# CGuerreroCordova/HydroDEM

Measured on AMD Instinct MI355X. Metric: Mcells/s sink-fill+D8 on 16384^2 float32 DEM, higher is better.
Workload: dtype f32; 1 GPU; 16384x16384 float32 synthetic DEM (SURVEY 8d 'rough': plane + 4 sinusoids + 0.5 m noise + 0.1% pits), SinkFill eps=0 to exact convergence + D8; 16384 rows per GPU, row-block partition; rows_per_gpu=16384, cols=16384, tiles=70225, visits_unchanged=25721, visits_flat=3352, certifying_rounds=0, halo_exchanges=0

## Files before the change

### hydrodem_amd/csrc/hdem_sinkfill.hip

```cpp
#include "hdem_internal.h"

#include <algorithm>
#include <cmath>
#include <cstdlib>

namespace {

constexpr int FT = 62;
constexpr int WN = 64;
constexpr int TS = WN + 1;
constexpr int NT = 64;
constexpr int ITER_MAX = 8;
constexpr int INIT_NT = 256;
constexpr int INIT_ROWS = 4;
constexpr int KEY_NONE = 0x7fffffff;
constexpr int SEED_KEYS = 1 << 20;
constexpr int AUX_SC1 = 16;
constexpr int COARSE_SHIFT = 4;
constexpr int HUB_EDGE = 4 * WN;
constexpr float HUB_BIG = 3.0e38f;
constexpr int HUB_MIN_TILES = 64;
constexpr int HUB_MIN_TILES_NESTED = 36;
constexpr int COARSE_MIN_CELLS = 6000 * 6000;
constexpr int PEND_SHARDS = 64;
// ... 131 lines not shown
        h_cur = h_next;
    }
}

__device__ __forceinline__ void transpose(float (&v)[WN], float *T, int lane)
{
#pragma unroll
    for (int i = 0; i < WN; ++i) T[i * TS + lane] = v[i];
    __syncthreads();
#pragma unroll
    for (int i = 0; i < WN; ++i) v[i] = T[lane * TS + i];
    __syncthreads();
}

__device__ __forceinline__ float wave_min(float v)
{
#pragma unroll
    for (int o = 32; o >= 1; o >>= 1) v = fminf(v, __shfl_xor(v, o));
    return v;
}

__device__ __forceinline__ int float_key(float f)
{
    int i = __builtin_bit_cast(int, f);
    return i ^ ((i >> 31) & 0x7fffffff);
}

#ifdef HDEM_VISIT_PROF
#define PROF_MARK(k) do { long long now_ = wall_clock64(); out.ticks[k] += now_ - tprof_; tprof_ = now_; } while (0)
#else
#define PROF_MARK(k) do { } while (0)
#endif

struct hub_bounds {
    float lv[9];
    bool mine;
};

struct visit_result {
#ifdef HDEM_VISIT_PROF
    long long ticks[6];
#endif
    bool changed;
    bool more;
    unsigned dirs;
    int iters;
    int flat_bits;
    int zmax_bits;
};

template <bool HAS_EPS, bool COHERENT>
__device__ __forceinline__ visit_result tile_visit(const float *__restrict__ zg, float *wg,
                                                   int H, int W, float eps, int ty, int tx,
                                                   float *T, uint8_t *d8 = nullptr,
                                                   float flat_level = HDEM_INF,
                                                   const hub_bounds *hb = nullptr)
{
    const int lane = threadIdx.x;
    const int y0 = ty * FT, x0 = tx * FT;
    const int x = x0 + lane;
#ifdef HDEM_VISIT_PROF
    const long long tprof_entry_ = wall_clock64();
#endif

    float z[WN], w[WN];
    const int xc = min(x, W - 1);
    float *wbase = wg + (size_t)y0 * W;
    const size_t wbytes = (size_t)(H - y0) * W * sizeof(float);
    const __amdgpu_buffer_rsrc_t wrsrc = __builtin_amdgcn_make_buffer_rsrc(
        wbase, 0, COHERENT ? (int)(unsigned)(wbytes < 0xffffffffull ? wbytes : 0xffffffffull) : 0,
        0x00020000);
    const int hbrow = H - 1 - y0;
    if (COHERENT) {
        const __amdgpu_buffer_rsrc_t zrsrc = __builtin_amdgcn_make_buffer_rsrc(
            const_cast<float *>(zg) + (size_t)y0 * W, 0,
            (int)(unsigned)(wbytes < 0xffffffffull ? wbytes : 0xffffffffull), 0x00020000);
        const unsigned col = (unsigned)xc * (unsigned)sizeof(float);
        const unsigned pitch = (unsigned)W * (unsigned)sizeof(float);
#pragma unroll
        for (int r = 0; r < WN; ++r) {
            const unsigned row = (unsigned)min(r, hbrow) * pitch;
            z[r] = __builtin_bit_cast(float, __builtin_amdgcn_raw_buffer_load_b32(zrsrc, col, row, 0));
            w[r] = __builtin_bit_cast(float, __builtin_amdgcn_raw_buffer_load_b32(wrsrc, col, row, AUX_SC1));
        }
    } else {
#pragma unroll
        for (int r = 0; r < WN; ++r) {
            const size_t o = (size_t)min(y0 + r, H - 1) * W + xc;
            z[r] = zg[o];
            w[r] = wg[o];
        }
    }
    const bool lane_pin = lane == 0 || lane == WN - 1 || x == 0 || x >= W - 1;
    const bool lane_out = x >= W;
    const bool partial = x0 + WN > W || y0 + WN > H;
    unsigned long long free_n = ~0ull, free_s = ~0ull;
    unsigned free_lo = 0, free_hi = 0;
    float hub_t = -HDEM_INF, hub_m = -HDEM_INF, hub_b = -HDEM_INF;
    if (COHERENT && hb) {
        const int k = lane == 0 ? 0 : (lane == WN - 1 ? 2 : 1);
        hub_t = k == 0 ? hb->lv[0] : (k == 1 ? hb->lv[1] : hb->lv[2]);
        hub_m = k == 0 ? hb->lv[3] : (k == 1 ? hb->lv[4] : hb->lv[5]);
        hub_b = k == 0 ? hb->lv[6] : (k == 1 ? hb->lv[7] : hb->lv[8]);
    }
    const int pin_from = lane_pin ? 0 : min(hbrow, WN - 1);
    const int raise_to = x >= W - 1 ? 0 : min(hbrow, WN);
#pragma unroll
    for (int r = 0; r < WN; ++r) {
        float wc = fminf(w[r], HDEM_INF), zc = fminf(z[r], HDEM_INF);
        if (COHERENT) {
            const float bound = r == 0 ? hub_t : (r == WN - 1 ? hub_b : hub_m);
            wc = fmaxf(wc, r < raise_to ? bound : -HDEM_INF);
        }
        if (!COHERENT && partial && (lane_out || y0 + r >= H)) { wc = HDEM_INF; zc = HDEM_INF; }
        if (COHERENT) {
            if (r == 0) free_n = __ballot(zc < wc);
            if (r == WN - 1) free_s = __ballot(zc < wc);
            if (r < 32) shift_in_less(free_lo, zc, wc);
            else shift_in_less(free_hi, zc, wc);
        }
        z[r] = (r == 0 || r == WN - 1 || r >= pin_from) ? wc : zc;
        w[r] = wc;
    }
    if (COHERENT && partial) {
        const unsigned long long in_lanes = __ballot(!lane_out);
        free_n &= in_lanes;
        free_s = hbrow >= WN - 1 ? (free_s & in_lanes) : 0ull;
    }

    if (COHERENT && flat_level < HDEM_INF) {
        const bool inner_lane = lane >= 2 && lane <= FT - 1;
#pragma unroll
        for (int r = 2; r <= FT - 1; ++r) w[r] = inner_lane ? flat_level : w[r];
    }

    unsigned long long free_w = 0, free_e = 0;
    if (COHERENT) {
        const unsigned wl = __builtin_amdgcn_readlane(free_lo, 0), wh = __builtin_amdgcn_readlane(free_hi, 0);
        const unsigned el = __builtin_amdgcn_readlane(free_lo, WN - 1), eh = __builtin_amdgcn_readlane(free_hi, WN - 1);
        free_w = ((unsigned long long)__builtin_bitreverse32(wh) << 32) | __builtin_bitreverse32(wl);
        free_e = ((unsigned long long)__builtin_bitreverse32(eh) << 32) | __builtin_bitreverse32(el);
        if (partial && hbrow < WN - 1) {
            const unsigned long long in_rows = (2ull << hbrow) - 1;
            free_w &= in_rows;
            free_e &= in_rows;
        }
    }
    visit_result out;
    out.flat_bits = out.zmax_bits = FLAT_NONE;
#ifdef HDEM_VISIT_PROF
    for (int k = 0; k < 6; ++k) out.ticks[k] = 0;
    long long tprof_ = tprof_entry_;
    asm volatile("s_waitcnt vmcnt(0)" ::: "memory");
    PROF_MARK(0);
#endif
    out.dirs = 0;
    out.iters = 0;
    scan_masks V = {0, 0, 0};
    check_rows<HAS_EPS>(z, w, eps, V);
    V.all |= V.first | V.last;
    bool more = V.all != 0;
    out.changed = more;
    const bool force_store = COHERENT && hb && hb->mine;
    const unsigned long long b1 = 1ull << 1, bl = 1ull << FT;
    unsigned long long mv_r1 = V.first, mv_r62 = V.last, mv_c1 = V.all & b1, mv_c62 = V.all & bl;
    PROF_MARK(1);
    if (more || force_store) {
        float zt[WN];
#pragma unroll
        for (int r = 0; r < WN; ++r) zt[r] = z[r];
        transpose(zt, T, lane);
        float r1_prev = w[1], r62_prev = w[FT];
        if (lane == 1 || lane == FT) {
            float *dst = T + (lane == 1 ? 0 : WN);
#pragma unroll
            for (int r = 0; r < WN; ++r) dst[r] = w[r];
        }
        __syncthreads();
        float c1_prev = T[lane], c62_prev = T[WN + lane];
        __syncthreads();
        float hl = HDEM_INF, hr = HDEM_INF;
        PROF_MARK(2);
        for (; out.iters < ITER_MAX && more; ++out.iters) {
            scan_lines<HAS_EPS>(z, w, eps);
            transpose(w, T, lane);
            hl = w[0];
            hr = w[WN - 1];
            or_changed(mv_c1, w[1], c1_prev);
            or_changed(mv_c62, w[FT], c62_prev);
            c1_prev = w[1];
            c62_prev = w[FT];
            scan_lines<HAS_EPS>(zt, w, eps);
            or_changed(mv_c1, w[1], c1_prev);
            or_changed(mv_c62, w[FT], c62_prev);
            c1_prev = w[1];
            c62_prev = w[FT];
// ... 299 lines not shown
                                                       bool changed, bool more, unsigned dirs,
                                                       int iters)
{
    const int lane = threadIdx.x;
    const int ty = t / tiles_x, tx = t - ty * tiles_x, slot = t / G, owner = t % G;
    int *my_state = state + (size_t)owner * S, *my_prio = prio + (size_t)owner * S;
    const int now_key = SEED_KEYS + (int)(wall_clock64() & 0x3fffffff);
    if (changed && dirs) {
        asm volatile("s_waitcnt vmcnt(0)" ::: "memory");
        if (lane < 8 && ((dirs >> lane) & 1u)) {
            const int t2 = neighbour_tile(lane, ty, tx, tiles_x, tiles_y);
            if (t2 >= 0) wake_async(t2, now_key, G, S, state, prio, pend);
        }
    }
    if (lane == 8) {
        if (more) atomicMin(&my_prio[slot], now_key);
        const int target = more ? ST_QUEUED : ST_IDLE;
        const int old = atomicCAS(&my_state[slot], ST_RUNNING, target);
        if (old == ST_DIRTY) atomicExch(&my_state[slot], ST_QUEUED);
        else if (target == ST_IDLE) atomicAdd(pend + (owner % PEND_SHARDS) * PEND_STRIDE, -1);
        add_stats(stats, b, changed, more, iters);
    }
}

struct flat_result {
    int handled;
    bool changed;
    unsigned dirs;
    float level;
};

__device__ __attribute__((noinline)) flat_result flat_visit(float *wg, int H, int W, int ty, int tx,
                                                            float L, float zmax,
                                                            const hub_bounds *hb)
{
    const int lane = threadIdx.x;
    const int y0 = ty * FT, x0 = tx * FT;
    float *wbase = wg + (size_t)y0 * W;
    const size_t wbytes = (size_t)(H - y0) * W * sizeof(float);
    const __amdgpu_buffer_rsrc_t wrsrc = __builtin_amdgcn_make_buffer_rsrc(
        wbase, 0, (int)(unsigned)(wbytes < 0xffffffffull ? wbytes : 0xffffffffull), 0x00020000);
    auto at = [&](int r, int c) { return (unsigned)(((size_t)r * W + x0 + c) * sizeof(float)); };
    auto ld = [&](unsigned off) {
        return fminf(__builtin_bit_cast(float, __builtin_amdgcn_raw_buffer_load_b32(
                         wrsrc, off, 0, AUX_SC1)), HDEM_INF);
    };
    float top = ld(at(0, lane)), bottom = ld(at(WN - 1, lane));
    float left = ld(at(lane, 0)), right = ld(at(lane, WN - 1));
    if (hb) {
        const int k = lane == 0 ? 0 : (lane == WN - 1 ? 2 : 1);
        top = fmaxf(top, k == 0 ? hb->lv[0] : (k == 1 ? hb->lv[1] : hb->lv[2]));
        bottom = fmaxf(bottom, k == 0 ? hb->lv[6] : (k == 1 ? hb->lv[7] : hb->lv[8]));
        left = fmaxf(left, k == 0 ? hb->lv[0] : (k == 1 ? hb->lv[3] : hb->lv[6]));
        right = fmaxf(right, k == 0 ? hb->lv[2] : (k == 1 ? hb->lv[5] : hb->lv[8]));
    }
    const float low = wave_min(fminf(fminf(top, bottom), fminf(left, right)));
    flat_result out = {1, false, 0u, L};
    if (low >= L) return out;
    if (low < zmax) { out.handled = 0; return out; }
    out.changed = true;
    out.level = low;
    const unsigned bits = __builtin_bit_cast(unsigned, low);
    if (lane >= 1 && lane <= FT) {
        __builtin_amdgcn_raw_buffer_store_b32(bits, wrsrc, at(1, lane), 0, AUX_SC1);
        __builtin_amdgcn_raw_buffer_store_b32(bits, wrsrc, at(FT, lane), 0, AUX_SC1);
        if (lane >= 2 && lane <= FT - 1) {
            __builtin_amdgcn_raw_buffer_store_b32(bits, wrsrc, at(lane, 1), 0, AUX_SC1);
            __builtin_amdgcn_raw_buffer_store_b32(bits, wrsrc, at(lane, FT), 0, AUX_SC1);
        }
    }
    const unsigned long long mid = ((1ull << FT) - 1) << 1, hi = 1ull << (WN - 1);
    const unsigned long long n = __ballot(top > low), s_ = __ballot(bottom > low);
    const unsigned long long w_ = __ballot(left > low), e = __ballot(right > low);
    if (n & 1ull) out.dirs |= 1u << 0;
    if (n & mid) out.dirs |= 1u << 1;
    if (n & hi) out.dirs |= 1u << 2;
    if (w_ & mid) out.dirs |= 1u << 3;
    if (e & mid) out.dirs |= 1u << 4;
    if (s_ & 1ull) out.dirs |= 1u << 5;
    if (s_ & mid) out.dirs |= 1u << 6;
    if (s_ & hi) out.dirs |= 1u << 7;
    return out;
}

__global__ __launch_bounds__(NT) void flat_store_kernel(float *wg, int H, int W, int tiles_x,
                                                        int ntiles, const int *__restrict__ flat,
                                                        const float *__restrict__ hub_lev,
                                                        const int *__restrict__ applied,
// ... 211 lines not shown
                                                          int *pend, int *error,
                                                          unsigned long long *stats,
                                                          long long budget_ticks, int soft,
                                                          int *flat, int *zmax,
                                                          const float *__restrict__ hub_lev,
                                                          int *applied,
                                                          const int *__restrict__ seam_words)
{
    __shared__ float T[WN * TS];
    if (seam_words && (seam_words[0] | seam_words[1] | seam_words[2]) == 0) return;
    const int G = gridDim.x, b = blockIdx.x;
    const long long t_begin = wall_clock64();
    if (threadIdx.x == 0) atomicAdd(error + 1, 1);
    while (ld_relaxed(error + 1) < G && ld_relaxed(error) == 0) {
        if (wall_clock64() - t_begin > 20000) {
            if (threadIdx.x == 0) atomicExch(error + 3, 1);
            break;
        }
        __builtin_amdgcn_s_sleep(8);
    }
    if (ld_relaxed(error) != 0) return;
    long long t_mark = t_begin, busy = 0, idle = 0;
    for (;;) {
        if (soft && wall_clock64() - t_begin > budget_ticks) break;
        const int t = __builtin_amdgcn_readfirstlane(
            async_pick(b, G, S, ntiles, state, prio, pend, soft ? error + 2 : error, t_begin,
                       budget_ticks));
        long long now = wall_clock64();
        idle += now - t_mark;
        t_mark = now;
        if (t < 0) break;
        const int ty = t / tiles_x, tx = t - ty * tiles_x;
        float flat_level = HDEM_INF;
        hub_bounds hb;
        bool use_hb = false, first_visit = false;
        const int fb_raw = HAS_EPS ? FLAT_NONE : ld_relaxed(flat + t);
        if (!HAS_EPS && hub_lev) {
            const int k9 = threadIdx.x < 9 ? (int)threadIdx.x : 4;
            const int ny = ty + k9 / 3 - 1, nx = tx + k9 % 3 - 1;
            const bool there = threadIdx.x < 9 && ny >= 0 && ny < tiles_y && nx >= 0 && nx < tiles_x;
            float l = -HDEM_INF;
            int seen = 1;
            if (there) {
                seen = ld_relaxed(applied + ny * tiles_x + nx);
                l = hub_lev[(size_t)(2 * ny + 1) * (2 * tiles_x + 1) + 2 * nx + 1];
            }
            l = (seen || l != l) ? -HDEM_INF : (l >= HUB_BIG ? HDEM_INF : l);
            first_visit = __builtin_amdgcn_readlane(seen, 4) == 0;
            use_hb = first_visit || __ballot(l > -HDEM_INF) != 0;
            if (use_hb) {
#pragma unroll
                for (int k = 0; k < 9; ++k)
                    hb.lv[k] = __builtin_bit_cast(
                        float, __builtin_amdgcn_readlane(__builtin_bit_cast(int, l), k));
                hb.mine = first_visit;
            }
            asm volatile("" ::: "memory");
        }
        if (!HAS_EPS) {
            const int fb = __builtin_amdgcn_readfirstlane(fb_raw);
            if (fb != FLAT_NONE) {
                flat_level = __builtin_bit_cast(float, fb);
                const float zm = __builtin_bit_cast(
                    float, __builtin_amdgcn_readfirstlane(ld_relaxed(zmax + t)));
                const flat_result f = flat_visit(wg, H, W, ty, tx, flat_level, zm,
                                                 use_hb ? &hb : nullptr);
                if (f.handled) {
                    if (f.changed) {
                        if (threadIdx.x == 0)
                            __hip_atomic_store(flat + t, __builtin_bit_cast(int, f.level),
                                               __ATOMIC_RELAXED, __HIP_MEMORY_SCOPE_AGENT);
                        asm volatile("s_waitcnt vmcnt(0)" ::: "memory");
                    }
                    async_finish(t, b, G, S, tiles_x, tiles_y, state, prio, pend, stats, f.changed,
                                 false, f.dirs, 0);
                    now = wall_clock64();
                    if (threadIdx.x == 8) {
                        stats[(size_t)b * STAT_WORDS + STAT_FLAT] += 1;
                        stats[(size_t)b * STAT_WORDS + STAT_FLAT_SAME] += f.changed ? 0 : 1;
                    }
                    busy += now - t_mark;
                    t_mark = now;
                    continue;
                }
            }
        }
        const visit_result v = tile_visit<HAS_EPS, true>(zg, wg, H, W, eps, ty, tx, T, nullptr,
                                                         flat_level, use_hb ? &hb : nullptr);
        if (first_visit) {
            asm volatile("s_waitcnt vmcnt(0)" ::: "memory");
            if (threadIdx.x == 0)
                __hip_atomic_store(applied + t, 1, __ATOMIC_RELAXED, __HIP_MEMORY_SCOPE_AGENT);
            asm volatile("s_waitcnt vmcnt(0)" ::: "memory");
        }
        if (!HAS_EPS && (v.flat_bits != FLAT_NONE || flat_level < HDEM_INF)) {
            if (threadIdx.x == 0) {
                __hip_atomic_store(flat + t, v.flat_bits, __ATOMIC_RELAXED, __HIP_MEMORY_SCOPE_AGENT);
                if (v.flat_bits != FLAT_NONE)
                    __hip_atomic_store(zmax + t, v.zmax_bits, __ATOMIC_RELAXED,
                                       __HIP_MEMORY_SCOPE_AGENT);
            }
            asm volatile("s_waitcnt vmcnt(0)" ::: "memory");
        }
#ifdef HDEM_VISIT_PROF
        const long long t_v = wall_clock64();
#endif
        async_finish(t, b, G, S, tiles_x, tiles_y, state, prio, pend, stats, v.changed, v.more,
                     v.dirs, v.iters);
        now = wall_clock64();
#ifdef HDEM_VISIT_PROF
        if (threadIdx.x == 8) {
            for (int k = 0; k < 6; ++k) stats[(size_t)b * STAT_WORDS + STAT_PROF + k] += v.ticks[k];
            stats[(size_t)b * STAT_WORDS + STAT_PROF + 6] += (unsigned long long)(now - t_v);
        }
#endif
        busy += now - t_mark;
        t_mark = now;
    }
    if (threadIdx.x == 0) {
        stats[(size_t)b * STAT_WORDS + 4] += (unsigned long long)busy;
        stats[(size_t)b * STAT_WORDS + 5] += (unsigned long long)idle;
// ... 824 lines not shown
```

### hydrodem_amd/csrc/hdem_stencil.hip

```cpp
#include "hdem_internal.h"

namespace {

constexpr int TW = 256;
constexpr int TH = 32;
template <typename T> struct tile_rows { static constexpr int value = sizeof(T) == 8 ? TH / 2 : TH; };
constexpr int LS = TW + 8;
constexpr int NT = 256;

__device__ __forceinline__ int reflect(int i, int n)
{
    while (i < 0 || i >= n) {
        if (i < 0) i = -i - 1;
        if (i >= n) i = 2 * n - 1 - i;
    }
    return i;
}

template <typename T, bool REFLECT>
__device__ __forceinline__ void stage_tile(const T *__restrict__ src, int H, int W,
                                           int y0, int x0, T *t)
{
    constexpr int THT = tile_rows<T>::value;
    constexpr int V = 16 / sizeof(T);
// ... 20 lines not shown
                int xx = gx + k;
                T e = T(0);
                if (REFLECT) e = src[(size_t)gy * W + reflect(xx, W)];
                else if (row_ok && xx < W) e = src[(size_t)gy * W + xx];
                v[j][k] = e;
            }
        }
    }
#pragma unroll
    for (int j = 0; j < CHUNKS; ++j) {
        const int i = tid + j * NT;
        if (i < (THT + 2) * CPR)
            *reinterpret_cast<vec_t *>(t + (i / CPR) * LS + 4 + (i % CPR) * V) = v[j];
    }
    for (int i = tid; i < (THT + 2) * 2; i += NT) {
        int r = i >> 1, side = i & 1;
        int gy = y0 - 1 + r, gx = side ? x0 + TW : x0 - 1;
        T e = T(0);
        if (REFLECT) e = src[(size_t)reflect(gy, H) * W + reflect(gx, W)];
        else if (gy >= 0 && gy < H && gx >= 0 && gx < W) e = src[(size_t)gy * W + gx];
        t[r * LS + (side ? 4 + TW : 3)] = e;
    }
}

template <typename T>
__device__ __forceinline__ void read_row6(const T *t, int r, int cg, T (&o)[6])
{
    const T *p = t + r * LS + 4 + 4 * cg;
    o[0] = p[-1];
    o[1] = p[0]; o[2] = p[1]; o[3] = p[2]; o[4] = p[3];
    o[5] = p[4];
}

__device__ __forceinline__ unsigned d8_code(float nw, float n, float ne, float w,
                                            float c, float e, float sw, float s,
                                            float se)
{
    const float dg = 0.70710678f;
    float best = 0.0f;
    unsigned code = 0;
    float d;
    d = (c - nw) * dg; if (d > best) { best = d; code = 32; }
    d = (c - n);       if (d > best) { best = d; code = 64; }
    d = (c - ne) * dg; if (d > best) { best = d; code = 128; }
    d = (c - w);       if (d > best) { best = d; code = 16; }
    d = (c - e);       if (d > best) { best = d; code = 1; }
    d = (c - sw) * dg; if (d > best) { best = d; code = 8; }
    d = (c - s);       if (d > best) { best = d; code = 4; }
    d = (c - se) * dg; if (d > best) { best = d; code = 2; }
    return code;
}

__global__ __launch_bounds__(NT) void d8_kernel(const float *__restrict__ z, int H,
                                               int W, uint8_t *__restrict__ out,
                                               int tiles_x, int vec_store)
{
    __shared__ __attribute__((aligned(16))) float t[(TH + 2) * LS];
    const int bx = blockIdx.x % tiles_x, by = blockIdx.x / tiles_x;
    const int x0 = bx * TW, y0 = by * TH;
    stage_tile<float, false>(z, H, W, y0, x0, t);
    __syncthreads();

    const int cg = threadIdx.x & 63, rg = threadIdx.x >> 6;
    const int x = x0 + 4 * cg;
    if (x >= W) return;
    float a[6], b[6], c[6];
    read_row6(t, rg * 8 + 0, cg, a);
    read_row6(t, rg * 8 + 1, cg, b);
#pragma unroll
    for (int rr = 0; rr < 8; ++rr) {
        const int y = y0 + rg * 8 + rr;
        read_row6(t, rg * 8 + rr + 2, cg, c);
        if (y < H) {
            unsigned code[4];
#pragma unroll
            for (int k = 0; k < 4; ++k) {
                unsigned cd = d8_code(a[k], a[k + 1], a[k + 2], b[k], b[k + 1],
                                      b[k + 2], c[k], c[k + 1], c[k + 2]);
                int xx = x + k;
                bool interior = y > 0 && y < H - 1 && xx > 0 && xx < W - 1;
                code[k] = interior ? cd : 0u;
            }
            uint8_t *o = out + (size_t)y * W + x;
            if (vec_store && x + 4 <= W) {
                *reinterpret_cast<uint32_t *>(o) =
                    code[0] | (code[1] << 8) | (code[2] << 16) | (code[3] << 24);
            } else {
#pragma unroll
                for (int k = 0; k < 4; ++k)
                    if (x + k < W) o[k] = (uint8_t)code[k];
            }
        }
#pragma unroll
        for (int k = 0; k < 6; ++k) { a[k] = b[k]; b[k] = c[k]; }
    }
}

template <bool HAS_EPS>
__global__ __launch_bounds__(NT) void certify_d8_kernel(const float *__restrict__ z,
                                                       const float *__restrict__ w, int H, int W,
                                                       float eps, uint8_t *__restrict__ out,
                                                       int tiles_x, int vec_store, int *flag)
{
    __shared__ __attribute__((aligned(16))) float t[(TH + 2) * LS];
    const int bx = blockIdx.x % tiles_x, by = blockIdx.x / tiles_x;
    const int x0 = bx * TW, y0 = by * TH;
    stage_tile<float, false>(w, H, W, y0, x0, t);
    __syncthreads();

    const int cg = threadIdx.x & 63, rg = threadIdx.x >> 6;
    const int x = x0 + 4 * cg;
    if (x >= W) return;
    float zc[8][4];
#pragma unroll
    for (int rr = 0; rr < 8; ++rr) {
        const int y = min(y0 + rg * 8 + rr, H - 1);
        if (x + 4 <= W) {
            const hdem_f4 m = hdem_ld4u(z + (size_t)y * W + x);
            zc[rr][0] = m[0]; zc[rr][1] = m[1]; zc[rr][2] = m[2]; zc[rr][3] = m[3];
        } else {
#pragma unroll
            for (int k = 0; k < 4; ++k) zc[rr][k] = z[(size_t)y * W + min(x + k, W - 1)];
        }
    }
    bool lower = false;
    float a[6], b[6], c[6];
    read_row6(t, rg * 8 + 0, cg, a);
    read_row6(t, rg * 8 + 1, cg, b);
#pragma unroll
    for (int rr = 0; rr < 8; ++rr) {
        const int y = y0 + rg * 8 + rr;
        read_row6(t, rg * 8 + rr + 2, cg, c);
        if (y < H) {
            unsigned code[4];
#pragma unroll
            for (int k = 0; k < 4; ++k) {
                const int xx = x + k;
                const bool interior = y > 0 && y < H - 1 && xx > 0 && xx < W - 1;
                float m = fminf(fminf(fminf(a[k], a[k + 1]), fminf(a[k + 2], b[k])),
                                fminf(fminf(b[k + 1], b[k + 2]), fminf(c[k], fminf(c[k + 1], c[k + 2]))));
                m = fminf(m, HDEM_INF);
                if (HAS_EPS) m += eps;
                const float wc = fminf(b[k + 1], HDEM_INF), zz = fminf(zc[rr][k], HDEM_INF);
                lower |= interior && __builtin_amdgcn_fmed3f(zz, wc, m) != wc;
                const unsigned cd = d8_code(a[k], a[k + 1], a[k + 2], b[k], b[k + 1], b[k + 2], c[k],
                                            c[k + 1], c[k + 2]);
                code[k] = interior ? cd : 0u;
            }
            if (out) {
                uint8_t *o = out + (size_t)y * W + x;
                if (vec_store && x + 4 <= W) {
                    *reinterpret_cast<uint32_t *>(o) =
                        code[0] | (code[1] << 8) | (code[2] << 16) | (code[3] << 24);
                } else {
#pragma unroll
                    for (int k = 0; k < 4; ++k)
                        if (x + k < W) o[k] = (uint8_t)code[k];
                }
            }
        }
#pragma unroll
        for (int k = 0; k < 6; ++k) { a[k] = b[k]; b[k] = c[k]; }
    }
    if (lower) *flag = 1;
}

template <typename T>
__device__ __forceinline__ T mean9(const T (&a)[6], const T (&b)[6], const T (&c)[6],
                                   int k, int do_round)
{
    double acc = 0.0;
    acc += (double)a[k]; acc += (double)a[k + 1]; acc += (double)a[k + 2];
    acc += (double)b[k]; acc += (double)b[k + 1]; acc += (double)b[k + 2];
    acc += (double)c[k]; acc += (double)c[k + 1]; acc += (double)c[k + 2];
    T s = (T)acc;
    T m = s / T(9);
    if (do_round) m = sizeof(T) == 4 ? (T)rintf((float)m) : (T)rint((double)m);
    return m;
}

template <typename T>
__global__ __launch_bounds__(NT) void boxmean3_kernel(const T *__restrict__ x, int H,
                                                     int W, T *__restrict__ out,
                                                     int tiles_x, int do_round)
{
    constexpr int THT = tile_rows<T>::value;
    constexpr int RPW = THT / 4;
    __shared__ __attribute__((aligned(16))) T t[(THT + 2) * LS];
    const int bx = blockIdx.x % tiles_x, by = blockIdx.x / tiles_x;
    const int x0 = bx * TW, y0 = by * THT;
    stage_tile<T, true>(x, H, W, y0, x0, t);
    __syncthreads();

    const int cg = threadIdx.x & 63, rg = threadIdx.x >> 6;
    const int xc = x0 + 4 * cg;
    if (xc >= W) return;
    T a[6], b[6], c[6];
// ... 38 lines not shown
    double acc = 0.0;
    for (int j = 0; j < kh; ++j) {
        int gy = reflect(y + j - py, H);
        for (int k = 0; k < kw; ++k) {
            double w = wt[(kh - 1 - j) * kw + (kw - 1 - k)];
            if (w != 0.0)
                acc += (double)x[(size_t)gy * W + reflect(xx + k - px, W)] * w;
        }
    }
    const T s = (T)acc;
    out[i] = s / (T)(kh * kw);
}

template <typename T>
__global__ __launch_bounds__(NT) void around_kernel(const T *x, int64_t n, T *out)
{
    int64_t i = (int64_t)blockIdx.x * NT + threadIdx.x;
    if (i < n) out[i] = sizeof(T) == 4 ? (T)rintf((float)x[i]) : (T)rint((double)x[i]);
}

inline int tiles_of(int H, int W, int th, int *tx)
{
    *tx = (W + TW - 1) / TW;
    return *tx * ((H + th - 1) / th);
}

}

int hdem_certify_d8_launch(hdem_ctx *ctx, const float *z, const float *w, int H, int W, float eps,
                           uint8_t *d8, int *flag)
{
    int tx, nt = tiles_of(H, W, TH, &tx);
    const int vec = d8 && (W % 4 == 0) && ((uintptr_t)d8 % 4 == 0);
    if (eps != 0.0f)
        hipLaunchKernelGGL(certify_d8_kernel<true>, dim3(nt), dim3(NT), 0, ctx->stream, z, w, H, W,
                           eps, d8, tx, vec, flag);
    else
        hipLaunchKernelGGL(certify_d8_kernel<false>, dim3(nt), dim3(NT), 0, ctx->stream, z, w, H, W,
                           eps, d8, tx, vec, flag);
    HDEM_HIP_CHECK(hipGetLastError());
    return HDEM_OK;
}

extern "C" int hdem_d8_f32_dev(hdem_ctx *ctx, const float *z, int H, int W, uint8_t *out)
{
    HDEM_REQUIRE(ctx, HDEM_ERR_BAD_ARG, "ctx is null");
    if (int rc = hdem_check_raster(z, out, H, W)) return rc;
    HDEM_HIP_CHECK(hipSetDevice(ctx->device));
    int tx, nt = tiles_of(H, W, TH, &tx);
    int vec = (W % 4 == 0) && ((uintptr_t)out % 4 == 0);
    {
        hdem_scoped_timer tm(ctx, HDEM_K_D8, (int64_t)H * W);
        hipLaunchKernelGGL(d8_kernel, dim3(nt), dim3(NT), 0, ctx->stream, z, H, W, out,
                           tx, vec);
    }
    HDEM_HIP_CHECK(hipGetLastError());
    return HDEM_OK;
}

extern "C" int hdem_d8_f32(hdem_ctx *ctx, const float *z, int H, int W, uint8_t *out)
{
    HDEM_REQUIRE(ctx, HDEM_ERR_BAD_ARG, "ctx is null");
    if (int rc = hdem_check_raster(z, out, H, W)) return rc;
    HDEM_HIP_CHECK(hipSetDevice(ctx->device));
    size_t n = (size_t)H * W;
    hdem_dbuf dz, dout;
    if (int rc = dz.alloc(ctx, n * sizeof(float))) return rc;
    if (int rc = dout.alloc(ctx, n)) return rc;
    if (int rc = hdem_memcpy_h2d(ctx, dz.p, z, n * sizeof(float))) return rc;
    if (int rc = hdem_d8_f32_dev(ctx, (const float *)dz.p, H, W, (uint8_t *)dout.p)) return rc;
    return hdem_memcpy_d2h(ctx, out, dout.p, n);
}
// ... 99 lines not shown
```

Before: 62230 Mcells/s.

## Prefetch z rows early, pass hub bounds in registers, branchless D8 code

The sink-fill worklist loop now issues the tile's z loads before hub-level decoding and flat handling, so their latency overlaps that work. Hub bounds are passed as per-lane registers picked with readlane instead of a 9-float struct, which avoids a local array. The D8 direction code becomes a branchless max-then-select chain. The certify kernel reuses horizontal row minima across rows and gets a template that skips D8 work when no output is requested. z may now be loaded twice when a flat visit falls through, and holding zpre raises register pressure.

```diff
diff --git a/hydrodem_amd/csrc/hdem_sinkfill.hip b/hydrodem_amd/csrc/hdem_sinkfill.hip
--- a/hydrodem_amd/csrc/hdem_sinkfill.hip
+++ b/hydrodem_amd/csrc/hdem_sinkfill.hip
@@ -187,10 +187,14 @@
 #define PROF_MARK(k) do { } while (0)
 #endif
 
-struct hub_bounds {
-    float lv[9];
-    bool mine;
-};
+__device__ __forceinline__ float hub_pick(float l, int a, int b, int c)
+{
+    const int lane = threadIdx.x;
+    const float la = __builtin_bit_cast(float, __builtin_amdgcn_readlane(__builtin_bit_cast(int, l), a));
+    const float lb = __builtin_bit_cast(float, __builtin_amdgcn_readlane(__builtin_bit_cast(int, l), b));
+    const float lc = __builtin_bit_cast(float, __builtin_amdgcn_readlane(__builtin_bit_cast(int, l), c));
+    return lane == 0 ? la : (lane == WN - 1 ? lc : lb);
+}
 
 struct visit_result {
 #ifdef HDEM_VISIT_PROF
@@ -204,12 +208,33 @@
     int zmax_bits;
 };
 
-template <bool HAS_EPS, bool COHERENT>
+__device__ __forceinline__ void load_z_rows(const float *__restrict__ zg, int H, int W, int ty,
+                                            int tx, float (&z)[WN])
+{
+    const int y0 = ty * FT, x0 = tx * FT;
+    const size_t zbytes = (size_t)(H - y0) * W * sizeof(float);
+    const __amdgpu_buffer_rsrc_t zrsrc = __builtin_amdgcn_make_buffer_rsrc(
+        const_cast<float *>(zg) + (size_t)y0 * W, 0,
+        (int)(unsigned)(zbytes < 0xffffffffull ? zbytes : 0xffffffffull), 0x00020000);
+    const unsigned col = (unsigned)min(x0 + (int)threadIdx.x, W - 1) * (unsigned)sizeof(float);
+    const unsigned pitch = (unsigned)W * (unsigned)sizeof(float);
+    const int hbrow = H - 1 - y0;
+#pragma unroll
+    for (int r = 0; r < WN; ++r)
+        z[r] = __builtin_bit_cast(float, __builtin_amdgcn_raw_buffer_load_b32(
+                                             zrsrc, col, (unsigned)min(r, hbrow) * pitch, 0));
+}
+
+template <bool HAS_EPS, bool COHERENT, bool ZPRE = false>
 __device__ __forceinline__ visit_result tile_visit(const float *__restrict__ zg, float *wg,
                                                    int H, int W, float eps, int ty, int tx,
                                                    float *T, uint8_t *d8 = nullptr,
                                                    float flat_level = HDEM_INF,
-                                                   const hub_bounds *hb = nullptr)
+                                                   float hub_t = -HDEM_INF,
+                                                   float hub_m = -HDEM_INF,
+                                                   float hub_b = -HDEM_INF,
+                                                   bool hub_mine = false,
+                                                   const float *zpre = nullptr)
 {
     const int lane = threadIdx.x;
     const int y0 = ty * FT, x0 = tx * FT;
@@ -227,15 +252,18 @@
         0x00020000);
     const int hbrow = H - 1 - y0;
     if (COHERENT) {
+        const size_t zbytes = ZPRE ? 0 : wbytes;
         const __amdgpu_buffer_rsrc_t zrsrc = __builtin_amdgcn_make_buffer_rsrc(
             const_cast<float *>(zg) + (size_t)y0 * W, 0,
-            (int)(unsigned)(wbytes < 0xffffffffull ? wbytes : 0xffffffffull), 0x00020000);
+            (int)(unsigned)(zbytes < 0xffffffffull ? zbytes : 0xffffffffull), 0x00020000);
         const unsigned col = (unsigned)xc * (unsigned)sizeof(float);
         const unsigned pitch = (unsigned)W * (unsigned)sizeof(float);
 #pragma unroll
         for (int r = 0; r < WN; ++r) {
             const unsigned row = (unsigned)min(r, hbrow) * pitch;
-            z[r] = __builtin_bit_cast(float, __builtin_amdgcn_raw_buffer_load_b32(zrsrc, col, row, 0));
+            if (!ZPRE)
+                z[r] = __builtin_bit_cast(float, __builtin_amdgcn_raw_buffer_load_b32(zrsrc, col, row, 0));
+            if (ZPRE) z[r] = zpre[r];
             w[r] = __builtin_bit_cast(float, __builtin_amdgcn_raw_buffer_load_b32(wrsrc, col, row, AUX_SC1));
         }
     } else {
@@ -251,13 +279,6 @@
     const bool partial = x0 + WN > W || y0 + WN > H;
     unsigned long long free_n = ~0ull, free_s = ~0ull;
     unsigned free_lo = 0, free_hi = 0;
-    float hub_t = -HDEM_INF, hub_m = -HDEM_INF, hub_b = -HDEM_INF;
-    if (COHERENT && hb) {
-        const int k = lane == 0 ? 0 : (lane == WN - 1 ? 2 : 1);
-        hub_t = k == 0 ? hb->lv[0] : (k == 1 ? hb->lv[1] : hb->lv[2]);
-        hub_m = k == 0 ? hb->lv[3] : (k == 1 ? hb->lv[4] : hb->lv[5]);
-        hub_b = k == 0 ? hb->lv[6] : (k == 1 ? hb->lv[7] : hb->lv[8]);
-    }
     const int pin_from = lane_pin ? 0 : min(hbrow, WN - 1);
     const int raise_to = x >= W - 1 ? 0 : min(hbrow, WN);
 #pragma unroll
@@ -316,7 +337,7 @@
     V.all |= V.first | V.last;
     bool more = V.all != 0;
     out.changed = more;
-    const bool force_store = COHERENT && hb && hb->mine;
+    const bool force_store = COHERENT && hub_mine;
     const unsigned long long b1 = 1ull << 1, bl = 1ull << FT;
     unsigned long long mv_r1 = V.first, mv_r62 = V.last, mv_c1 = V.all & b1, mv_c62 = V.all & bl;
     PROF_MARK(1);
@@ -682,7 +703,8 @@
 
 __device__ __attribute__((noinline)) flat_result flat_visit(float *wg, int H, int W, int ty, int tx,
                                                             float L, float zmax,
-                                                            const hub_bounds *hb)
+                                                            float hub_top, float hub_bottom,
+                                                            float hub_left, float hub_right)
 {
     const int lane = threadIdx.x;
     const int y0 = ty * FT, x0 = tx * FT;
@@ -697,13 +719,10 @@
     };
     float top = ld(at(0, lane)), bottom = ld(at(WN - 1, lane));
     float left = ld(at(lane, 0)), right = ld(at(lane, WN - 1));
-    if (hb) {
-        const int k = lane == 0 ? 0 : (lane == WN - 1 ? 2 : 1);
-        top = fmaxf(top, k == 0 ? hb->lv[0] : (k == 1 ? hb->lv[1] : hb->lv[2]));
-        bottom = fmaxf(bottom, k == 0 ? hb->lv[6] : (k == 1 ? hb->lv[7] : hb->lv[8]));
-        left = fmaxf(left, k == 0 ? hb->lv[0] : (k == 1 ? hb->lv[3] : hb->lv[6]));
-        right = fmaxf(right, k == 0 ? hb->lv[2] : (k == 1 ? hb->lv[5] : hb->lv[8]));
-    }
+    top = fmaxf(top, hub_top);
+    bottom = fmaxf(bottom, hub_bottom);
+    left = fmaxf(left, hub_left);
+    right = fmaxf(right, hub_right);
     const float low = wave_min(fminf(fminf(top, bottom), fminf(left, right)));
     flat_result out = {1, false, 0u, L};
     if (low >= L) return out;
@@ -981,29 +1000,28 @@
         if (t < 0) break;
         const int ty = t / tiles_x, tx = t - ty * tiles_x;
         float flat_level = HDEM_INF;
-        hub_bounds hb;
-        bool use_hb = false, first_visit = false;
+        bool first_visit = false;
+        float hub_l = -HDEM_INF;
         const int fb_raw = HAS_EPS ? FLAT_NONE : ld_relaxed(flat + t);
-        if (!HAS_EPS && hub_lev) {
+        const bool hub = !HAS_EPS && hub_lev;
+        float l = -HDEM_INF;
+        int seen = 1;
+        if (hub) {
             const int k9 = threadIdx.x < 9 ? (int)threadIdx.x : 4;
             const int ny = ty + k9 / 3 - 1, nx = tx + k9 % 3 - 1;
             const bool there = threadIdx.x < 9 && ny >= 0 && ny < tiles_y && nx >= 0 && nx < tiles_x;
-            float l = -HDEM_INF;
-            int seen = 1;
             if (there) {
                 seen = ld_relaxed(applied + ny * tiles_x + nx);
                 l = hub_lev[(size_t)(2 * ny + 1) * (2 * tiles_x + 1) + 2 * nx + 1];
             }
+        }
+        constexpr bool Z_EARLY = !HAS_EPS;
+        float zpre[WN];
+        if (Z_EARLY) load_z_rows(zg, H, W, ty, tx, zpre);
+        if (hub) {
             l = (seen || l != l) ? -HDEM_INF : (l >= HUB_BIG ? HDEM_INF : l);
             first_visit = __builtin_amdgcn_readlane(seen, 4) == 0;
-            use_hb = first_visit || __ballot(l > -HDEM_INF) != 0;
-            if (use_hb) {
-#pragma unroll
-                for (int k = 0; k < 9; ++k)
-                    hb.lv[k] = __builtin_bit_cast(
-                        float, __builtin_amdgcn_readlane(__builtin_bit_cast(int, l), k));
-                hb.mine = first_visit;
-            }
+            hub_l = l;
             asm volatile("" ::: "memory");
         }
         if (!HAS_EPS) {
@@ -1013,7 +1031,8 @@
                 const float zm = __builtin_bit_cast(
                     float, __builtin_amdgcn_readfirstlane(ld_relaxed(zmax + t)));
                 const flat_result f = flat_visit(wg, H, W, ty, tx, flat_level, zm,
-                                                 use_hb ? &hb : nullptr);
+                                                 hub_pick(hub_l, 0, 1, 2), hub_pick(hub_l, 6, 7, 8),
+                                                 hub_pick(hub_l, 0, 3, 6), hub_pick(hub_l, 2, 5, 8));
                 if (f.handled) {
                     if (f.changed) {
                         if (threadIdx.x == 0)
@@ -1032,10 +1051,12 @@
                     t_mark = now;
                     continue;
                 }
+                if (Z_EARLY) load_z_rows(zg, H, W, ty, tx, zpre);
             }
         }
-        const visit_result v = tile_visit<HAS_EPS, true>(zg, wg, H, W, eps, ty, tx, T, nullptr,
-                                                         flat_level, use_hb ? &hb : nullptr);
+        const visit_result v = tile_visit<HAS_EPS, true, Z_EARLY>(
+            zg, wg, H, W, eps, ty, tx, T, nullptr, flat_level, hub_pick(hub_l, 0, 1, 2),
+            hub_pick(hub_l, 3, 4, 5), hub_pick(hub_l, 6, 7, 8), first_visit, zpre);
         if (first_visit) {
             asm volatile("s_waitcnt vmcnt(0)" ::: "memory");
             if (threadIdx.x == 0)
diff --git a/hydrodem_amd/csrc/hdem_stencil.hip b/hydrodem_amd/csrc/hdem_stencil.hip
--- a/hydrodem_amd/csrc/hdem_stencil.hip
+++ b/hydrodem_amd/csrc/hdem_stencil.hip
@@ -78,21 +78,39 @@
 
 __device__ __forceinline__ unsigned d8_code(float nw, float n, float ne, float w,
                                             float c, float e, float sw, float s,
-                                            float se)
+                                            float se, bool keep = true)
 {
     const float dg = 0.70710678f;
-    float best = 0.0f;
+    const float d0 = (c - nw) * dg, d1 = c - n, d2 = (c - ne) * dg, d3 = c - w;
+    const float d4 = c - e, d5 = (c - sw) * dg, d6 = c - s, d7 = (c - se) * dg;
+    float best = fmaxf(fmaxf(0.0f, d0), d1);
+    best = fmaxf(fmaxf(best, d2), d3);
+    best = fmaxf(fmaxf(best, d4), d5);
+    best = fmaxf(fmaxf(best, d6), d7);
     unsigned code = 0;
-    float d;
-    d = (c - nw) * dg; if (d > best) { best = d; code = 32; }
-    d = (c - n);       if (d > best) { best = d; code = 64; }
-    d = (c - ne) * dg; if (d > best) { best = d; code = 128; }
-    d = (c - w);       if (d > best) { best = d; code = 16; }
-    d = (c - e);       if (d > best) { best = d; code = 1; }
-    d = (c - sw) * dg; if (d > best) { best = d; code = 8; }
-    d = (c - s);       if (d > best) { best = d; code = 4; }
-    d = (c - se) * dg; if (d > best) { best = d; code = 2; }
-    return code;
+    code = d7 == best ? 2u : code;
+    code = d6 == best ? 4u : code;
+    code = d5 == best ? 8u : code;
+    code = d4 == best ? 1u : code;
+    code = d3 == best ? 16u : code;
+    code = d2 == best ? 128u : code;
+    code = d1 == best ? 64u : code;
+    code = d0 == best ? 32u : code;
+    return (keep && best > 0.0f) ? code : 0u;
+}
+
+__device__ __forceinline__ void store_codes(uint8_t *__restrict__ out, int W, int y, int x,
+                                            int vec_store, const unsigned (&code)[4])
+{
+    uint8_t *o = out + (size_t)y * W + x;
+    if (vec_store && x + 4 <= W) {
+        *reinterpret_cast<uint32_t *>(o) =
+            code[0] | (code[1] << 8) | (code[2] << 16) | (code[3] << 24);
+    } else {
+#pragma unroll
+        for (int k = 0; k < 4; ++k)
+            if (x + k < W) o[k] = (uint8_t)code[k];
+    }
 }
 
 __global__ __launch_bounds__(NT) void d8_kernel(const float *__restrict__ z, int H,
@@ -105,9 +123,12 @@
     stage_tile<float, false>(z, H, W, y0, x0, t);
     __syncthreads();
 
-    const int cg = threadIdx.x & 63, rg = threadIdx.x >> 6;
+    const int cg = threadIdx.x & 63, rg = __builtin_amdgcn_readfirstlane(threadIdx.x >> 6);
     const int x = x0 + 4 * cg;
     if (x >= W) return;
+    bool col_in[4];
+#pragma unroll
+    for (int k = 0; k < 4; ++k) col_in[k] = (x + k > 0) & (x + k < W - 1);
     float a[6], b[6], c[6];
     read_row6(t, rg * 8 + 0, cg, a);
     read_row6(t, rg * 8 + 1, cg, b);
@@ -115,32 +136,19 @@
     for (int rr = 0; rr < 8; ++rr) {
         const int y = y0 + rg * 8 + rr;
         read_row6(t, rg * 8 + rr + 2, cg, c);
-        if (y < H) {
-            unsigned code[4];
-#pragma unroll
-            for (int k = 0; k < 4; ++k) {
-                unsigned cd = d8_code(a[k], a[k + 1], a[k + 2], b[k], b[k + 1],
-                                      b[k + 2], c[k], c[k + 1], c[k + 2]);
-                int xx = x + k;
-                bool interior = y > 0 && y < H - 1 && xx > 0 && xx < W - 1;
-                code[k] = interior ? cd : 0u;
-            }
-            uint8_t *o = out + (size_t)y * W + x;
-            if (vec_store && x + 4 <= W) {
-                *reinterpret_cast<uint32_t *>(o) =
-                    code[0] | (code[1] << 8) | (code[2] << 16) | (code[3] << 24);
-            } else {
-#pragma unroll
-                for (int k = 0; k < 4; ++k)
-                    if (x + k < W) o[k] = (uint8_t)code[k];
-            }
-        }
+        const bool row_in = (y > 0) & (y < H - 1);
+        unsigned code[4];
+#pragma unroll
+        for (int k = 0; k < 4; ++k)
+            code[k] = d8_code(a[k], a[k + 1], a[k + 2], b[k], b[k + 1], b[k + 2], c[k],
+                              c[k + 1], c[k + 2], row_in & col_in[k]);
+        if (y < H) store_codes(out, W, y, x, vec_store, code);
 #pragma unroll
         for (int k = 0; k < 6; ++k) { a[k] = b[k]; b[k] = c[k]; }
     }
 }
 
-template <bool HAS_EPS>
+template <bool HAS_EPS, bool WITH_D8>
 __global__ __launch_bounds__(NT) void certify_d8_kernel(const float *__restrict__ z,
                                                        const float *__restrict__ w, int H, int W,
                                                        float eps, uint8_t *__restrict__ out,
@@ -152,7 +160,7 @@
     stage_tile<float, false>(w, H, W, y0, x0, t);
     __syncthreads();
 
-    const int cg = threadIdx.x & 63, rg = threadIdx.x >> 6;
+    const int cg = threadIdx.x & 63, rg = __builtin_amdgcn_readfirstlane(threadIdx.x >> 6);
     const int x = x0 + 4 * cg;
     if (x >= W) return;
     float zc[8][4];
@@ -167,44 +175,42 @@
             for (int k = 0; k < 4; ++k) zc[rr][k] = z[(size_t)y * W + min(x + k, W - 1)];
         }
     }
+    bool col_in[4];
+#pragma unroll
+    for (int k = 0; k < 4; ++k) col_in[k] = (x + k > 0) & (x + k < W - 1);
     bool lower = false;
     float a[6], b[6], c[6];
+    float ha[4], hb[4], hc[4];
     read_row6(t, rg * 8 + 0, cg, a);
     read_row6(t, rg * 8 + 1, cg, b);
+#pragma unroll
+    for (int k = 0; k < 4; ++k) {
+        ha[k] = fminf(fminf(a[k], a[k + 1]), a[k + 2]);
+        hb[k] = fminf(fminf(b[k], b[k + 1]), b[k + 2]);
+    }
 #pragma unroll
     for (int rr = 0; rr < 8; ++rr) {
         const int y = y0 + rg * 8 + rr;
         read_row6(t, rg * 8 + rr + 2, cg, c);
-        if (y < H) {
-            unsigned code[4];
-#pragma unroll
-            for (int k = 0; k < 4; ++k) {
-                const int xx = x + k;
-                const bool interior = y > 0 && y < H - 1 && xx > 0 && xx < W - 1;
-                float m = fminf(fminf(fminf(a[k], a[k + 1]), fminf(a[k + 2], b[k])),
-                                fminf(fminf(b[k + 1], b[k + 2]), fminf(c[k], fminf(c[k + 1], c[k + 2]))));
-                m = fminf(m, HDEM_INF);
-                if (HAS_EPS) m += eps;
-                const float wc = fminf(b[k + 1], HDEM_INF), zz = fminf(zc[rr][k], HDEM_INF);
-                lower |= interior && __builtin_amdgcn_fmed3f(zz, wc, m) != wc;
-                const unsigned cd = d8_code(a[k], a[k + 1], a[k + 2], b[k], b[k + 1], b[k + 2], c[k],
-                                            c[k + 1], c[k + 2]);
-                code[k] = interior ? cd : 0u;
-            }
-            if (out) {
-                uint8_t *o = out + (size_t)y * W + x;
-                if (vec_store && x + 4 <= W) {
-                    *reinterpret_cast<uint32_t *>(o) =
-                        code[0] | (code[1] << 8) | (code[2] << 16) | (code[3] << 24);
-                } else {
-#pragma unroll
-                    for (int k = 0; k < 4; ++k)
-                        if (x + k < W) o[k] = (uint8_t)code[k];
-                }
-            }
+        const bool row_in = (y > 0) & (y < H - 1);
+        unsigned code[4];
+#pragma unroll
+        for (int k = 0; k < 4; ++k) {
+            const bool interior = row_in & col_in[k];
+            hc[k] = fminf(fminf(c[k], c[k + 1]), c[k + 2]);
+            float m = fminf(fminf(fminf(ha[k], hb[k]), hc[k]), HDEM_INF);
+            if (HAS_EPS) m += eps;
+            const float wc = fminf(b[k + 1], HDEM_INF), zz = fminf(zc[rr][k], HDEM_INF);
+            lower |= interior & (__builtin_amdgcn_fmed3f(zz, wc, m) != wc);
+            if (WITH_D8)
+                code[k] = d8_code(a[k], a[k + 1], a[k + 2], b[k], b[k + 1], b[k + 2], c[k],
+                                  c[k + 1], c[k + 2], interior);
         }
+        if (WITH_D8 && y < H) store_codes(out, W, y, x, vec_store, code);
 #pragma unroll
         for (int k = 0; k < 6; ++k) { a[k] = b[k]; b[k] = c[k]; }
+#pragma unroll
+        for (int k = 0; k < 4; ++k) { ha[k] = hb[k]; hb[k] = hc[k]; }
     }
     if (lower) *flag = 1;
 }
@@ -311,12 +317,9 @@
 {
     int tx, nt = tiles_of(H, W, TH, &tx);
     const int vec = d8 && (W % 4 == 0) && ((uintptr_t)d8 % 4 == 0);
-    if (eps != 0.0f)
-        hipLaunchKernelGGL(certify_d8_kernel<true>, dim3(nt), dim3(NT), 0, ctx->stream, z, w, H, W,
-                           eps, d8, tx, vec, flag);
-    else
-        hipLaunchKernelGGL(certify_d8_kernel<false>, dim3(nt), dim3(NT), 0, ctx->stream, z, w, H, W,
-                           eps, d8, tx, vec, flag);
+    auto kernel = eps != 0.0f ? (d8 ? certify_d8_kernel<true, true> : certify_d8_kernel<true, false>)
+                              : (d8 ? certify_d8_kernel<false, true> : certify_d8_kernel<false, false>);
+    hipLaunchKernelGGL(kernel, dim3(nt), dim3(NT), 0, ctx->stream, z, w, H, W, eps, d8, tx, vec, flag);
     HDEM_HIP_CHECK(hipGetLastError());
     return HDEM_OK;
 }
```

Result: faster. 62950 Mcells/s (median of 6 runs) (+1.2%).

## Share D8 drop computations across rows and specialize interior tiles

Applied to the files above, without the earlier changes.

D8 slope differences are now computed once per row pair and reused: the downward drops of one row become the upward drops of the next, with the sign flipped. In the certify kernel, the 3x3 minimum is built from per-row horizontal min3 values that slide down the tile. Whole-wave ballots skip D8 code generation for rows where no cell sits above its neighbourhood minimum. Interior tiles get a template variant with no edge checks and a wave-uniform row index. The aim is fewer ALU ops and branches in the stencil, at the cost of more registers and template instantiations.

```diff
diff --git a/hydrodem_amd/csrc/hdem_stencil.hip b/hydrodem_amd/csrc/hdem_stencil.hip
--- a/hydrodem_amd/csrc/hdem_stencil.hip
+++ b/hydrodem_amd/csrc/hdem_stencil.hip
@@ -76,23 +76,144 @@
     o[5] = p[4];
 }
 
-__device__ __forceinline__ unsigned d8_code(float nw, float n, float ne, float w,
-                                            float c, float e, float sw, float s,
-                                            float se)
+struct d8_down {
+    float s[4];
+    float se[5];
+    float sw[5];
+};
+
+__device__ __forceinline__ void d8_down_drops(const float (&u)[6], const float (&d)[6], d8_down &o)
 {
     const float dg = 0.70710678f;
-    float best = 0.0f;
-    unsigned code = 0;
+#pragma unroll
+    for (int k = 0; k < 4; ++k) o.s[k] = u[k + 1] - d[k + 1];
+#pragma unroll
+    for (int j = 0; j < 5; ++j) {
+        o.se[j] = (u[j] - d[j + 1]) * dg;
+        o.sw[j] = (u[j + 1] - d[j]) * dg;
+    }
+}
+
+__device__ __forceinline__ void d8_code_upper(const d8_down &up, const float (&e)[5], int k,
+                                              float &best, unsigned &code)
+{
+    float x, nb = 0.0f;
+    code = 0;
+    x = up.se[k];     if (x < nb) { nb = x; code = 32; }
+    x = up.s[k];      if (x < nb) { nb = x; code = 64; }
+    x = up.sw[k + 1]; if (x < nb) { nb = x; code = 128; }
+    x = e[k];         if (x < nb) { nb = x; code = 16; }
+    best = -nb;
+    x = e[k + 1];     if (x > best) { best = x; code = 1; }
+}
+__device__ __forceinline__ void d8_code_lower(const d8_down &dn, int k, float &best,
+                                              unsigned &code)
+{
     float d;
-    d = (c - nw) * dg; if (d > best) { best = d; code = 32; }
-    d = (c - n);       if (d > best) { best = d; code = 64; }
-    d = (c - ne) * dg; if (d > best) { best = d; code = 128; }
-    d = (c - w);       if (d > best) { best = d; code = 16; }
-    d = (c - e);       if (d > best) { best = d; code = 1; }
-    d = (c - sw) * dg; if (d > best) { best = d; code = 8; }
-    d = (c - s);       if (d > best) { best = d; code = 4; }
-    d = (c - se) * dg; if (d > best) { best = d; code = 2; }
-    return code;
+    d = dn.sw[k];      if (d > best) { best = d; code = 8; }
+    d = dn.s[k];       if (d > best) { best = d; code = 4; }
+    d = dn.se[k + 1];  if (d > best) { best = d; code = 2; }
+}
+
+__device__ __forceinline__ void row_min3(const float (&r)[6], float (&h)[4])
+{
+#pragma unroll
+    for (int k = 0; k < 4; ++k) h[k] = fminf(fminf(r[k], r[k + 1]), r[k + 2]);
+}
+
+template <bool CERT, bool HAS_EPS, bool EDGE>
+__device__ __forceinline__ void d8_stream_rows(const float *t, const float *__restrict__ z, int H,
+                                               int W, int y0, int x0, float eps,
+                                               uint8_t *__restrict__ out, int vec_store, int *flag)
+{
+    const int cg = threadIdx.x & 63;
+    const int rg = __builtin_amdgcn_readfirstlane(threadIdx.x >> 6);
+    const int x = x0 + 4 * cg;
+    if (EDGE && x >= W) return;
+    float zc[CERT ? 8 : 1][4];
+    if (CERT) {
+#pragma unroll
+        for (int rr = 0; rr < 8; ++rr) {
+            const int y = EDGE ? min(y0 + rg * 8 + rr, H - 1) : y0 + rg * 8 + rr;
+            if (!EDGE || x + 4 <= W) {
+                const hdem_f4 m = hdem_ld4u(z + (size_t)y * W + x);
+                zc[rr][0] = m[0]; zc[rr][1] = m[1]; zc[rr][2] = m[2]; zc[rr][3] = m[3];
+            } else {
+#pragma unroll
+                for (int k = 0; k < 4; ++k) zc[rr][k] = z[(size_t)y * W + min(x + k, W - 1)];
+            }
+        }
+    }
+    const bool want = !CERT || out;
+    unsigned long long lower = 0;
+    float b[6], c[6], ha[4], hb[4], hc[4];
+    d8_down up, dn;
+    read_row6(t, rg * 8 + 0, cg, c);
+    read_row6(t, rg * 8 + 1, cg, b);
+    if (want) d8_down_drops(c, b, up);
+    if (CERT) { row_min3(c, ha); row_min3(b, hb); }
+#pragma unroll
+    for (int rr = 0; rr < 8; ++rr) {
+        const int y = y0 + rg * 8 + rr;
+        read_row6(t, rg * 8 + rr + 2, cg, c);
+        if (CERT) row_min3(c, hc);
+        if (want) d8_down_drops(b, c, dn);
+        if (!EDGE || y < H) {
+            const bool row_in = !EDGE || (y > 0 && y < H - 1);
+            bool skip = false;
+            if (CERT) {
+                bool below = false, low = false;
+#pragma unroll
+                for (int k = 0; k < 4; ++k) {
+                    float m = fminf(fminf(fminf(ha[k], hb[k]), hc[k]), HDEM_INF);
+                    below |= m < b[k + 1];
+                    if (HAS_EPS) m += eps;
+                    const float wc = fminf(b[k + 1], HDEM_INF), zz = fminf(zc[rr][k], HDEM_INF);
+                    const bool interior = row_in && (!EDGE || (x + k > 0 && x + k < W - 1));
+                    low |= interior && __builtin_amdgcn_fmed3f(zz, wc, m) != wc;
+                }
+                lower |= __ballot(low);
+                skip = !want || __ballot(below) == 0;
+            }
+            unsigned code[4] = {0u, 0u, 0u, 0u};
+            if (!skip) {
+                float e[5], best[4];
+#pragma unroll
+                for (int j = 0; j < 5; ++j) e[j] = b[j] - b[j + 1];
+#pragma unroll
+                for (int k = 0; k < 4; ++k) {
+                    d8_code_upper(up, e, k, best[k], code[k]);
+                    d8_code_lower(dn, k, best[k], code[k]);
+                    const bool interior = row_in && (!EDGE || (x + k > 0 && x + k < W - 1));
+                    code[k] = interior ? code[k] : 0u;
+                }
+            }
+            if (want) {
+                uint8_t *o = out + (size_t)y * W + x;
+                if (!EDGE || (vec_store && x + 4 <= W)) {
+                    *reinterpret_cast<uint32_t *>(o) =
+                        code[0] | (code[1] << 8) | (code[2] << 16) | (code[3] << 24);
+                } else {
+#pragma unroll
+                    for (int k = 0; k < 4; ++k)
+                        if (x + k < W) o[k] = (uint8_t)code[k];
+                }
+            }
+        }
+        up = dn;
+#pragma unroll
+        for (int k = 0; k < 6; ++k) b[k] = c[k];
+        if (CERT) {
+#pragma unroll
+            for (int k = 0; k < 4; ++k) { ha[k] = hb[k]; hb[k] = hc[k]; }
+        }
+    }
+    if (CERT && lower) *flag = 1;
+}
+
+__device__ __forceinline__ bool tile_inside(int H, int W, int y0, int x0)
+{
+    return y0 > 0 && y0 + TH <= H - 1 && x0 > 0 && x0 + TW <= W - 1;
 }
 
 __global__ __launch_bounds__(NT) void d8_kernel(const float *__restrict__ z, int H,
@@ -104,40 +225,10 @@
     const int x0 = bx * TW, y0 = by * TH;
     stage_tile<float, false>(z, H, W, y0, x0, t);
     __syncthreads();
-
-    const int cg = threadIdx.x & 63, rg = threadIdx.x >> 6;
-    const int x = x0 + 4 * cg;
-    if (x >= W) return;
-    float a[6], b[6], c[6];
-    read_row6(t, rg * 8 + 0, cg, a);
-    read_row6(t, rg * 8 + 1, cg, b);
-#pragma unroll
-    for (int rr = 0; rr < 8; ++rr) {
-        const int y = y0 + rg * 8 + rr;
-        read_row6(t, rg * 8 + rr + 2, cg, c);
-        if (y < H) {
-            unsigned code[4];
-#pragma unroll
-            for (int k = 0; k < 4; ++k) {
-                unsigned cd = d8_code(a[k], a[k + 1], a[k + 2], b[k], b[k + 1],
-                                      b[k + 2], c[k], c[k + 1], c[k + 2]);
-                int xx = x + k;
-                bool interior = y > 0 && y < H - 1 && xx > 0 && xx < W - 1;
-                code[k] = interior ? cd : 0u;
-            }
-            uint8_t *o = out + (size_t)y * W + x;
-            if (vec_store && x + 4 <= W) {
-                *reinterpret_cast<uint32_t *>(o) =
-                    code[0] | (code[1] << 8) | (code[2] << 16) | (code[3] << 24);
-            } else {
-#pragma unroll
-                for (int k = 0; k < 4; ++k)
-                    if (x + k < W) o[k] = (uint8_t)code[k];
-            }
-        }
-#pragma unroll
-        for (int k = 0; k < 6; ++k) { a[k] = b[k]; b[k] = c[k]; }
-    }
+    if (vec_store && tile_inside(H, W, y0, x0))
+        d8_stream_rows<false, false, false>(t, nullptr, H, W, y0, x0, 0.0f, out, 1, nullptr);
+    else
+        d8_stream_rows<false, false, true>(t, nullptr, H, W, y0, x0, 0.0f, out, vec_store, nullptr);
 }
 
 template <bool HAS_EPS>
@@ -151,62 +242,10 @@
     const int x0 = bx * TW, y0 = by * TH;
     stage_tile<float, false>(w, H, W, y0, x0, t);
     __syncthreads();
-
-    const int cg = threadIdx.x & 63, rg = threadIdx.x >> 6;
-    const int x = x0 + 4 * cg;
-    if (x >= W) return;
-    float zc[8][4];
-#pragma unroll
-    for (int rr = 0; rr < 8; ++rr) {
-        const int y = min(y0 + rg * 8 + rr, H - 1);
-        if (x + 4 <= W) {
-            const hdem_f4 m = hdem_ld4u(z + (size_t)y * W + x);
-            zc[rr][0] = m[0]; zc[rr][1] = m[1]; zc[rr][2] = m[2]; zc[rr][3] = m[3];
-        } else {
-#pragma unroll
-            for (int k = 0; k < 4; ++k) zc[rr][k] = z[(size_t)y * W + min(x + k, W - 1)];
-        }
-    }
-    bool lower = false;
-    float a[6], b[6], c[6];
-    read_row6(t, rg * 8 + 0, cg, a);
-    read_row6(t, rg * 8 + 1, cg, b);
-#pragma unroll
-    for (int rr = 0; rr < 8; ++rr) {
-        const int y = y0 + rg * 8 + rr;
-        read_row6(t, rg * 8 + rr + 2, cg, c);
-        if (y < H) {
-            unsigned code[4];
-#pragma unroll
-            for (int k = 0; k < 4; ++k) {
-                const int xx = x + k;
-                const bool interior = y > 0 && y < H - 1 && xx > 0 && xx < W - 1;
-                float m = fminf(fminf(fminf(a[k], a[k + 1]), fminf(a[k + 2], b[k])),
-                                fminf(fminf(b[k + 1], b[k + 2]), fminf(c[k], fminf(c[k + 1], c[k + 2]))));
-                m = fminf(m, HDEM_INF);
-                if (HAS_EPS) m += eps;
-                const float wc = fminf(b[k + 1], HDEM_INF), zz = fminf(zc[rr][k], HDEM_INF);
-                lower |= interior && __builtin_amdgcn_fmed3f(zz, wc, m) != wc;
-                const unsigned cd = d8_code(a[k], a[k + 1], a[k + 2], b[k], b[k + 1], b[k + 2], c[k],
-                                            c[k + 1], c[k + 2]);
-                code[k] = interior ? cd : 0u;
-            }
-            if (out) {
-                uint8_t *o = out + (size_t)y * W + x;
-                if (vec_store && x + 4 <= W) {
-                    *reinterpret_cast<uint32_t *>(o) =
-                        code[0] | (code[1] << 8) | (code[2] << 16) | (code[3] << 24);
-                } else {
-#pragma unroll
-                    for (int k = 0; k < 4; ++k)
-                        if (x + k < W) o[k] = (uint8_t)code[k];
-                }
-            }
-        }
-#pragma unroll
-        for (int k = 0; k < 6; ++k) { a[k] = b[k]; b[k] = c[k]; }
-    }
-    if (lower) *flag = 1;
+    if ((vec_store || !out) && tile_inside(H, W, y0, x0))
+        d8_stream_rows<true, HAS_EPS, false>(t, z, H, W, y0, x0, eps, out, 1, flag);
+    else
+        d8_stream_rows<true, HAS_EPS, true>(t, z, H, W, y0, x0, eps, out, vec_store, flag);
 }
 
 template <typename T>
```

After: 62030 Mcells/s before, 61980 Mcells/s after. No clear change (-0.1%).
